# mnigm2001/Software-Defined-Radio

Measured on AMD Instinct MI355X. Metric: I/Q MS/s through front-end FIR+decimate+demod(+audio) per job; % HBM roofline, higher is better.
Workload: dtype i8+f32

## Files before the change

### software-defined-radio_amd/csrc/capi.hip

```cpp
#include "fmrx_internal.hpp"
#include "rds_station.hpp"
#include "build_id.hpp"

namespace fmrx {

static thread_local char g_err[512] = "";

void set_error(const char *fmt, ...)
{
    va_list ap;
    va_start(ap, fmt);
    vsnprintf(g_err, sizeof(g_err), fmt, ap);
    va_end(ap);
}

int fail(int code, const char *fmt, ...)
{
    va_list ap;
    va_start(ap, fmt);
    vsnprintf(g_err, sizeof(g_err), fmt, ap);
    va_end(ap);
    return code;
}

// ... 365 lines not shown
}

int fmrx_all_pass(const float *in, size_t n, float *state, size_t nstate, float *out)
{
    if (!in || !state || !out) return fail(FMRX_EINVAL, "all_pass: null buffer");
    if (n < nstate) return fail(FMRX_EINVAL, "all_pass: block of %zu samples shorter than the delay %zu", n, nstate);
    FMRX_TRY(require_device());
    Scratch &s = scratch();
    FMRX_TRY(s.a.ensure(n));
    FMRX_TRY(s.b.ensure(nstate));
    FMRX_TRY(s.c.ensure(n));
    FMRX_TRY(h2d(s.a.p, in, n * sizeof(float)));
    FMRX_TRY(h2d(s.b.p, state, nstate * sizeof(float)));
    FMRX_TRY(k_all_pass(s.a.p, n, s.b.p, nstate, s.c.p, nullptr));
    FMRX_TRY(d2h(out, s.c.p, n * sizeof(float)));
    std::memcpy(state, in + n - nstate, nstate * sizeof(float));
    return FMRX_OK;
}

int fmrx_fm_pll(const float *in, size_t n, float *nco_out, float *state, float freq, float Fs, float ncoScale,
                float phaseAdjust, float normBandwidth)
{
    if (!in || !nco_out || !state) return fail(FMRX_EINVAL, "fm_pll: null buffer");
    if (!(Fs > 0)) return fail(FMRX_EINVAL, "fm_pll: Fs must be positive");
    FMRX_TRY(require_device());
    Scratch &s = scratch();
    FMRX_TRY(s.a.ensure(n));
    FMRX_TRY(s.b.ensure(n + 1));
    FMRX_TRY(s.c.ensure(6));
    FMRX_TRY(h2d(s.a.p, in, n * sizeof(float)));
    FMRX_TRY(h2d(s.c.p, state, 6 * sizeof(float)));
    FMRX_TRY(k_fm_pll(s.a.p, n, s.b.p, s.c.p, freq, Fs, ncoScale, phaseAdjust, normBandwidth, 0, nullptr));
    FMRX_TRY(d2h(nco_out, s.b.p, (n + 1) * sizeof(float)));
    return d2h(state, s.c.p, 6 * sizeof(float));
}

int fmrx_stereo_mix(const float *stereo_filt, const float *pll, size_t n, float *mixer)
{
    if ((!stereo_filt || !pll || !mixer) && n) return fail(FMRX_EINVAL, "stereo_mix: null buffer");
    FMRX_TRY(require_device());
    Scratch &s = scratch();
    FMRX_TRY(s.a.ensure(n));
    FMRX_TRY(s.b.ensure(n));
    FMRX_TRY(s.c.ensure(n));
    FMRX_TRY(h2d(s.a.p, stereo_filt, n * sizeof(float)));
    FMRX_TRY(h2d(s.b.p, pll, n * sizeof(float)));
    FMRX_TRY(k_mix(s.a.p, s.b.p, n, s.c.p, nullptr));
    return d2h(mixer, s.c.p, n * sizeof(float));
}

int fmrx_stereo_combine(const float *stereo_final, const float *mono, size_t n, float *left, float *right)
{
    if ((!stereo_final || !mono || !left || !right) && n) return fail(FMRX_EINVAL, "stereo_combine: null buffer");
    FMRX_TRY(require_device());
    Scratch &s = scratch();
    FMRX_TRY(s.a.ensure(n));
    FMRX_TRY(s.b.ensure(n));
    FMRX_TRY(s.c.ensure(n));
    FMRX_TRY(s.d.ensure(n));
    FMRX_TRY(h2d(s.a.p, stereo_final, n * sizeof(float)));
    FMRX_TRY(h2d(s.b.p, mono, n * sizeof(float)));
    FMRX_TRY(k_combine(s.a.p, s.b.p, n, s.c.p, s.d.p, nullptr));
    FMRX_TRY(d2h(left, s.c.p, n * sizeof(float)));
    return d2h(right, s.d.p, n * sizeof(float));
}

int fmrx_diag_libm(int fn, const float *a, const float *b, size_t n, float *out)
{
    if (fn < 0 || fn > 5) return fail(FMRX_EINVAL, "diag_libm: fn must be 0 (sinf), 1 (cosf), 2 (atan2f) or 3..5 (their branch-free forms)");
    if ((!a || !out || (fn % 3 == 2 && !b)) && n) return fail(FMRX_EINVAL, "diag_libm: null buffer");
    FMRX_TRY(require_device());
    Scratch &s = scratch();
    FMRX_TRY(s.a.ensure(n));
    FMRX_TRY(s.b.ensure(n));
    FMRX_TRY(s.c.ensure(n));
    FMRX_TRY(h2d(s.a.p, a, n * sizeof(float)));
    if (fn % 3 == 2) FMRX_TRY(h2d(s.b.p, b, n * sizeof(float)));
    FMRX_TRY(k_libm_eval(fn, s.a.p, s.b.p, n, s.c.p, nullptr));
    return d2h(out, s.c.p, n * sizeof(float));
}

int fmrx_diag_stream_read_dev(const void *d_buf, size_t bytes, int method, void *stream)
{
    if (!d_buf || method < 0 || method > 4096) return fail(FMRX_EINVAL, "diag_stream_read_dev: bad arguments");
    FMRX_TRY(require_device());
    static thread_local DevBuf<unsigned> sink;
    FMRX_TRY(sink.ensure(4));
    return k_stream_read(d_buf, bytes, method, sink.p, static_cast<hipStream_t>(stream));
}

int fmrx_estimate_psd(float *freq, float *psd, const float *samples, size_t n, float Fs, int nfft)
{
    if (!freq || !psd || !samples) return fail(FMRX_EINVAL, "estimate_psd: null buffer");
    if (nfft < 2 || nfft % 2 || nfft > 65536) return fail(FMRX_EINVAL, "estimate_psd: nfft must be even and in 2..65536");
    if (n < static_cast<size_t>(nfft)) return fail(FMRX_EINVAL, "estimate_psd: %zu samples < nfft %d", n, nfft);
    if (!(Fs > 0)) return fail(FMRX_EINVAL, "estimate_psd: Fs must be positive");
    FMRX_TRY(require_device());
    Scratch &s = scratch();
    const size_t nseg = n / nfft, half = nfft / 2;
    FMRX_TRY(s.a.ensure(n));
    FMRX_TRY(s.b.ensure(nseg * half));
    FMRX_TRY(s.c.ensure(half));
    FMRX_TRY(s.d.ensure(half));
    FMRX_TRY(h2d(s.a.p, samples, nseg * nfft * sizeof(float)));
    FMRX_TRY(k_estimate_psd(s.a.p, n, Fs, nfft, s.b.p, s.c.p, s.d.p, nullptr));
    FMRX_TRY(d2h(freq, s.c.p, half * sizeof(float)));
    return d2h(psd, s.d.p, half * sizeof(float));
}

struct fmrx_fe_plan {
    FePlan plan;
};

int fmrx_fe_plan_create(fmrx_fe_plan **out, const float *h, size_t taps, unsigned decim)
{
    if (!out || !h) return fail(FMRX_EINVAL, "fe_plan_create: null argument");
    if (taps < 2 || taps > 65535) return fail(FMRX_EINVAL, "fe_plan_create: taps %zu not in 2..65535", taps);
    if (decim == 0) return fail(FMRX_EINVAL, "fe_plan_create: decim must be >= 1");
    FMRX_TRY(require_device());
    fmrx_fe_plan *p = new fmrx_fe_plan;
    int rc = fe_plan_init(p->plan, h, static_cast<int>(taps), static_cast<int>(decim));
    if (rc != FMRX_OK) {
        delete p;
        return rc;
    }
    *out = p;
    return FMRX_OK;
}

int fmrx_fe_plan_destroy(fmrx_fe_plan *plan)
{
    delete plan;
    return FMRX_OK;
}

int fmrx_fe_plan_is_specialised(const fmrx_fe_plan *plan) { return plan && plan->plan.fast ? 1 : 0; }
size_t fmrx_fe_plan_history_bytes(const fmrx_fe_plan *plan) { return plan ? plan->plan.hist_bytes : 0; }

int fmrx_fe_run_dev(const fmrx_fe_plan *plan, const uint8_t *d_iq, size_t n_samples, const uint8_t *d_hist, float *d_if,
                    int force_generic, void *stream)
{
    if (!plan || !d_iq || !d_if) return fail(FMRX_EINVAL, "fe_run_dev: null argument");
    return fe_launch(plan->plan, d_iq, n_samples, d_hist, d_if, default_options(), static_cast<hipStream_t>(stream),
                     force_generic != 0);
}

int fmrx_fe_fir_decim_u8(const uint8_t *iq, size_t n_samples, const float *h, size_t taps, unsigned decim, uint8_t *hist,
                         float *if_i, float *if_q, int force_generic)
{
    if (!iq || !h) return fail(FMRX_EINVAL, "fe_fir_decim_u8: null buffer");
    if (taps < 2 || taps > 65535) return fail(FMRX_EINVAL, "fe_fir_decim_u8: taps %zu not in 2..65535", taps);
    if (decim == 0) return fail(FMRX_EINVAL, "fe_fir_decim_u8: decim must be >= 1");
    if (hist && n_samples < taps - 1)
        return fail(FMRX_EINVAL, "fe_fir_decim_u8: block of %zu samples shorter than taps-1 = %zu", n_samples, taps - 1);
    FMRX_TRY(require_device());
    FePlan plan;
    FMRX_TRY(fe_plan_init(plan, h, static_cast<int>(taps), static_cast<int>(decim)));
    Scratch &s = scratch();
    const size_t n_out = n_samples / decim;
    const size_t hb = plan.hist_bytes, live = 2 * (taps - 1);
    FMRX_TRY(s.u.ensure(2 * n_samples));
    FMRX_TRY(s.uh.ensure(hb));
    FMRX_TRY(s.a.ensure(2 * n_out));
    FMRX_TRY(s.b.ensure(n_out));
    FMRX_TRY(s.c.ensure(n_out));
    FMRX_TRY(h2d(s.u.p, iq, 2 * n_samples));
    if (hist) {
// ... 88 lines not shown
```

### software-defined-radio_amd/csrc/kernels_diag.hip

```cpp
#include "fmrx_internal.hpp"

namespace fmrx {
namespace {

typedef unsigned u4 __attribute__((ext_vector_type(4)));

__global__ __launch_bounds__(256) void read_regs_kernel(const u4 *__restrict__ x, long n16, unsigned *__restrict__ out)
{
    const int lane = threadIdx.x & 63;
    const long waves = static_cast<long>(gridDim.x) * 4, w = static_cast<long>(blockIdx.x) * 4 + (threadIdx.x >> 6);
    const long pieces = n16 / 64;
    const long per = (pieces + waves - 1) / waves;
    const long p0 = w * per, p1 = p0 + per < pieces ? p0 + per : pieces;
    u4 acc = {0, 0, 0, 0};
    for (long p = p0; p < p1; p += 4) {
        u4 v[4];
#pragma unroll
        for (int i = 0; i < 4; i++) {
            const long q = p + i < p1 ? p + i : p1 - 1;
            v[i] = __builtin_nontemporal_load(x + q * 64 + lane);
        }
#pragma unroll
        for (int i = 0; i < 4; i++) acc ^= v[i];
    }
    if ((acc.x ^ acc.y ^ acc.z ^ acc.w) == 0x12345678u) out[0] = 1;
}

__global__ __launch_bounds__(256) void read_dma_kernel(const unsigned char *__restrict__ x, long n_bytes, unsigned *__restrict__ out, int SWEEP)
{
    extern __shared__ __attribute__((aligned(16))) unsigned char lds[];
    const int lane = threadIdx.x & 63, wave = threadIdx.x >> 6;
    unsigned char *ring = lds + wave * 4 * 3072;
    const long waves = static_cast<long>(gridDim.x) * 4, w = static_cast<long>(blockIdx.x) * 4 + wave;
    const long steps = n_bytes / 3072, per = (steps + waves - 1) / waves;
    const long s0 = w * per, s1 = s0 + per < steps ? s0 + per : steps;
    auto issue = [&](long s, int slot) {
        if (SWEEP) {
            const long i = s - s0, c = i / SWEEP, r = i - c * SWEEP;
            const long t = (c * waves + w) * SWEEP + r;
            s = t < steps ? t : steps - 1;
        }
#pragma unroll
        for (int k = 0; k < 3; k++)
            __builtin_amdgcn_global_load_lds((const __attribute__((address_space(1))) void *)(x + s * 3072 + k * 1024 + lane * 16),
                                             (__attribute__((address_space(3))) void *)(ring + slot * 3072 + k * 1024), 16, 0, 0);
    };
    u4 acc = {0, 0, 0, 0};
    for (int i = 0; i < 3 && s0 + i < s1; i++) issue(s0 + i, i);
    int slot = 0, fill = 3;
    for (long s = s0; s < s1; s++) {
        const bool steady = s + 3 < s1;
        if (steady) issue(s + 3, fill);
        if (steady) asm volatile("s_waitcnt vmcnt(9)" ::: "memory");
        else asm volatile("s_waitcnt vmcnt(0)" ::: "memory");
        const u4 *src = reinterpret_cast<const u4 *>(ring + slot * 3072);
        acc ^= src[lane] ^ src[64 + lane] ^ src[128 + lane];
        asm volatile("s_waitcnt lgkmcnt(0)" ::: "memory");
        slot = (slot + 1) & 3;
        fill = (fill + 1) & 3;
    }
    if ((acc.x ^ acc.y ^ acc.z ^ acc.w) == 0x12345678u) out[0] = 1;
}

}

int k_stream_read(const void *d_buf, size_t bytes, int method, unsigned *d_sink, hipStream_t s)
{
    if (bytes < 3072 * 1024) return fail(FMRX_EINVAL, "stream_read: buffer too small to mean anything");
    if (reinterpret_cast<uintptr_t>(d_buf) % 16) return fail(FMRX_EINVAL, "stream_read: buffer must be 16-byte aligned");
    if (method == 0)
        hipLaunchKernelGGL(read_regs_kernel, dim3(1024), dim3(256), 0, s, static_cast<const u4 *>(d_buf), static_cast<long>(bytes / 16), d_sink);
    else if (method == 1)
        hipLaunchKernelGGL(read_dma_kernel, dim3(512), dim3(256), 4 * 4 * 3072, s, static_cast<const unsigned char *>(d_buf),
                           static_cast<long>(bytes - bytes % 3072), d_sink, 0);
    else
        hipLaunchKernelGGL(read_dma_kernel, dim3(512), dim3(256), 4 * 4 * 3072, s, static_cast<const unsigned char *>(d_buf),
                           static_cast<long>(bytes - bytes % 3072), d_sink, method - 1);
    hipError_t e = hipGetLastError();
    if (e != hipSuccess) return fail(FMRX_EHIP, "launch stream_read: %s", hipGetErrorString(e));
    return FMRX_OK;
}

}
```

### software-defined-radio_amd/csrc/kernels_fe_mfma.hip

```cpp
#include "device_math.hpp"
#include "fe_mfma_host.hpp"
#include "fmrx_internal.hpp"

#include <cmath>
#include <type_traits>
#include <utility>

namespace fmrx {
namespace {

using i4 = int __attribute__((ext_vector_type(4)));
using f2 = float __attribute__((ext_vector_type(2)));
using f4 = float __attribute__((ext_vector_type(4)));

constexpr int iclamp(int v, int lo, int hi) { return v < lo ? lo : (v > hi ? hi : v); }

template <int T, int D, int PF = 0>
struct MfCfg {
    static constexpr int COL_OUT = 8;
    static constexpr int COLS = 16;
    static constexpr int TILE_OUT = COL_OUT * (COLS - 1);
    static constexpr int COL_BYTES = 2 * D * COL_OUT;
    static constexpr int STRIDE_BYTES = COL_BYTES * (COLS - 1);
    static constexpr int FRONT = (2 * (T - 1) + 15) / 16 * 16;
    static constexpr int WIN = FRONT + 2 * D * (COL_OUT - 1) + 2;
    static constexpr int KSTEPS = (WIN + 63) / 64;
    static constexpr int NDIG = kFeMfmaDigits;
    static constexpr int LEAD = COL_BYTES + FRONT;
    static constexpr int TILE_WIN = COL_BYTES * (COLS - 1) + 64 * KSTEPS;
    static constexpr int NPF = TILE_WIN / 1024;
    static constexpr int REM_LANES = (TILE_WIN % 1024) / 16;
    static constexpr int NP = NPF + (REM_LANES ? 1 : 0);
    static constexpr int SLOT = NP * 1024;
    static constexpr int P = PF ? PF : iclamp(8192 / TILE_WIN, 2, 8);
    static constexpr int NSLOT = P + 1;
    static constexpr int RING = NSLOT * SLOT;
    static_assert(TILE_WIN % 16 == 0 && COL_BYTES % 16 == 0, "16-byte fragments");
    static constexpr int YOUNGER = NP * P;
    static_assert(YOUNGER + 2 * P <= 63, "vmcnt is 6 bits");
};

template <class Fn, int... K>
__device__ __forceinline__ void for_each_index(std::integer_sequence<int, K...>, Fn &&f)
{
    (f(std::integral_constant<int, K>{}), ...);
}

template <int N>
__device__ __forceinline__ void wait_vmcnt()
{
    asm volatile("s_waitcnt vmcnt(%0)" ::"n"(N) : "memory");
}

template <int NPF, int REM_LANES>
__device__ __forceinline__ void dma_window(const uint8_t *__restrict__ x, const uint8_t *__restrict__ hist_end, long n_bytes,
                                           long s0, uint8_t *dst, int lane)
{
    constexpr int NP = NPF + (REM_LANES ? 1 : 0);
    if (s0 >= 0 && s0 + NP * 1024L <= n_bytes) {
        const uint8_t *base = x + s0;
#pragma unroll
        for (int k = 0; k < NP; k++)
            if (k < NPF || lane < REM_LANES)
                __builtin_amdgcn_global_load_lds((const __attribute__((address_space(1))) void *)(base + (lane * 16 + k * 1024)),
                                                 (__attribute__((address_space(3))) void *)(dst + k * 1024), 16, 0, 0);
    } else {
#pragma unroll
        for (int k = 0; k < NP; k++)
            if (k < NPF || lane < REM_LANES) {
                long off = s0 + k * 1024 + lane * 16;
                if (off > n_bytes - 16) off = n_bytes - 16;
                const uint8_t *src = off < 0 ? hist_end + off : x + off;
                __builtin_amdgcn_global_load_lds((const __attribute__((address_space(1))) void *)src,
                                                 (__attribute__((address_space(3))) void *)(dst + k * 1024), 16, 0, 0);
            }
    }
}

template <class C>
__device__ __forceinline__ void mf_dma_tile(const uint8_t *__restrict__ x, const uint8_t *__restrict__ hist_end, long n_bytes,
                                            int tile, uint8_t *ring, int rs, int lane)
{
    dma_window<C::NPF, C::REM_LANES>(x, hist_end, n_bytes, static_cast<long>(tile) * C::STRIDE_BYTES - C::LEAD,
                                     ring + rs * C::SLOT, lane);
}

template <int T, int D, int MINB, int PF>
__global__ __launch_bounds__(256, MINB) void fe_mfma_kernel(
    const uint8_t *__restrict__ x, const uint8_t *__restrict__ hist_end, long n_bytes, const i4 *__restrict__ a_img,
    float scale_lo, const float2 *__restrict__ prev_in, float *__restrict__ demod, float *__restrict__ y_if,
    float2 *__restrict__ prev_out, long n_out, int n_tiles, uint8_t *__restrict__ hist_next, int hist_bytes,
    const float *__restrict__ dhist_src, float *__restrict__ dhist_dst, int dhist_n)
{
    using C = MfCfg<T, D, PF>;
    extern __shared__ __attribute__((aligned(16))) uint8_t lds_raw[];
    const int lane = threadIdx.x & 63;
    const int wave = __builtin_amdgcn_readfirstlane(static_cast<int>(threadIdx.x >> 6));
    uint8_t *ring = lds_raw + wave * C::RING;
    const int tstep = static_cast<int>(gridDim.x) * 4;
    int tile = __builtin_amdgcn_readfirstlane(static_cast<int>(blockIdx.x) * 4 + wave);

    if (hist_next && tile == 0)
        for (int i = lane; i < hist_bytes; i += 64) hist_next[i] = x[n_bytes - hist_bytes + i];
    if (dhist_dst && tile == 1)
        for (int i = lane; i < dhist_n; i += 64) dhist_dst[i] = dhist_src[i];
    if (tile >= n_tiles) return;

    i4 a[C::KSTEPS][C::NDIG];
#pragma unroll
    for (int j = 0; j < C::KSTEPS; j++)
#pragma unroll
        for (int d = 0; d < C::NDIG; d++) a[j][d] = a_img[(j * C::NDIG + d) * 64 + lane];
    float ovi = 0.0f, ovq = 0.0f;
    const bool override_prev = prev_in != nullptr;
    if (override_prev) {
        const float2 p = *prev_in;
        ovi = p.x;
        ovq = p.y;
    }
    asm volatile("s_waitcnt vmcnt(0)" ::: "memory");
#pragma unroll
    for (int j = 0; j < C::KSTEPS; j++)
#pragma unroll
        for (int d = 0; d < C::NDIG; d++) asm volatile("" : "+v"(a[j][d]));
    asm volatile("" : "+v"(ovi), "+v"(ovq));

#pragma unroll
    for (int k = 0; k < C::P; k++)
        if (tile + k * tstep < n_tiles) mf_dma_tile<C>(x, hist_end, n_bytes, tile + k * tstep, ring, k, lane);

    const int col = lane & 15, g = lane >> 4;
    const int lane_off = C::COL_BYTES * col + 16 * g;
    const float scale_hi = scale_lo * 65536.0f;
    const bool with_if = y_if != nullptr;
    const int src_lane = lane >= 16 ? lane - 16 : lane + 47;
    int slot = 0, fill = C::P;
    auto fast_tile = [&](auto uc, auto modec, int t) {
        constexpr int u = decltype(uc)::value;
        constexpr int MODE = decltype(modec)::value;
        constexpr int FILL = (u + C::P) % C::NSLOT;
        {
            const uint8_t *src = x + (static_cast<long>(t + C::P * tstep) * C::STRIDE_BYTES - C::LEAD);
            uint8_t *dst = ring + FILL * C::SLOT;
#pragma unroll
            for (int q = 0; q < C::NP; q++)
                if (q < C::NPF || lane < C::REM_LANES)
                    __builtin_amdgcn_global_load_lds((const __attribute__((address_space(1))) void *)(src + (lane * 16 + q * 1024)),
                                                     (__attribute__((address_space(3))) void *)(dst + q * 1024), 16, 0, 0);
        }
        wait_vmcnt<C::YOUNGER + (MODE == 3 ? 2 : 1) * C::P>();
        __builtin_amdgcn_fence(__ATOMIC_ACQUIRE, "wavefront");
        __builtin_amdgcn_wave_barrier();
        const uint8_t *bsrc = ring + u * C::SLOT + lane_off;
        i4 b[C::KSTEPS];
#pragma unroll
        for (int j = 0; j < C::KSTEPS; j++) b[j] = *reinterpret_cast<const i4 *>(bsrc + 64 * j);
        __builtin_amdgcn_s_waitcnt(0xC07F);
// ... 164 lines not shown
        for (int d = 0; d < C::NDIG; d++) a[j][d] = a_img[(j * C::NDIG + d) * 64 + lane];
    asm volatile("s_waitcnt vmcnt(0)" ::: "memory");
#pragma unroll
    for (int j = 0; j < C::KSTEPS; j++)
#pragma unroll
        for (int d = 0; d < C::NDIG; d++) asm volatile("" : "+v"(a[j][d]));
    auto dma = [&](int t, int rs) {
        const int c = t / bk.tiles_per_row, j = t - c * bk.tiles_per_row;
        const long s0 = c * bk.in_pitch + bk.in_off + static_cast<long>(j) * C::STRIDE_BYTES - C::LEAD;
        dma_window<C::NPF, C::REM_LANES>(x, x, n_bytes, s0, ring + rs * C::SLOT, lane);
    };
#pragma unroll
    for (int k = 0; k < C::P; k++)
        if (tile + k * tstep < n_tiles) dma(tile + k * tstep, k);
    const int col = lane & 15, g = lane >> 4;
    const int lane_off = C::COL_BYTES * col + 16 * g;
    const float scale_hi = scale_lo * 65536.0f;
    const int src_lane = lane >= 16 ? lane - 16 : lane + 47;
    int slot = 0, fill = C::P;
    for (int it = 0; tile < n_tiles; tile += tstep, it++) {
        const bool steady = tile + C::P * tstep < n_tiles;
        if (steady) dma(tile + C::P * tstep, fill);
        if (steady) {
            if (it < C::P) wait_vmcnt<C::YOUNGER>();
            else wait_vmcnt<C::YOUNGER + C::P>();
        } else {
            wait_vmcnt<0>();
        }
        __builtin_amdgcn_fence(__ATOMIC_ACQUIRE, "wavefront");
        __builtin_amdgcn_wave_barrier();
        const uint8_t *bsrc = ring + slot * C::SLOT + lane_off;
        i4 b[C::KSTEPS];
#pragma unroll
        for (int j = 0; j < C::KSTEPS; j++) b[j] = *reinterpret_cast<const i4 *>(bsrc + 64 * j);
        __builtin_amdgcn_s_waitcnt(0xC07F);
        __builtin_amdgcn_fence(__ATOMIC_RELEASE, "wavefront");
        __builtin_amdgcn_wave_barrier();
        i4 acc[C::NDIG];
#pragma unroll
        for (int d = 0; d < C::NDIG; d++) acc[d] = (i4){0, 0, 0, 0};
#pragma unroll
        for (int j = 0; j < C::KSTEPS; j++) {
            const i4 bs = b[j] ^ static_cast<int>(0x80808080u);
#pragma unroll
            for (int d = 0; d < C::NDIG; d++) acc[d] = __builtin_amdgcn_mfma_i32_16x16x64_i8(a[j][d], bs, acc[d], 0, 0, 0);
        }
        float v[4];
#pragma unroll
        for (int k = 0; k < 4; k++) {
            int lo = acc[0][k];
            if (C::NDIG >= 2) lo += acc[1][k] * 256;
            const float flo = static_cast<float>(lo) * scale_lo;
            v[k] = C::NDIG >= 3 ? __builtin_fmaf(static_cast<float>(acc[2][k]), scale_hi, flo) : flo;
        }
        const float pi = __shfl(v[2], src_lane, 64), pq = __shfl(v[3], src_lane, 64);
        const float d0 = demod_fast(v[0], v[1], pi, pq), d1 = demod_fast(v[2], v[3], v[0], v[1]);
        const int c = tile / bk.tiles_per_row, j = tile - c * bk.tiles_per_row;
        const long ol = static_cast<long>(j) * C::TILE_OUT + C::COL_OUT * (col - 1) + 2 * g;
        if (col > 0 && ol < bk.n_row) *reinterpret_cast<f2 *>(demod + c * bk.out_pitch + bk.out_off + ol) = (f2){d0, d1};
        slot = slot + 1 == C::NSLOT ? 0 : slot + 1;
        fill = fill + 1 == C::NSLOT ? 0 : fill + 1;
    }
}

template <int T, int D, int TA, int DA>
struct FuCfg {
    using F = MfCfg<T, D>;
    static constexpr int TILE_OUT = 128;
    static constexpr int TILE_BYTES = F::COL_BYTES * 16;
    static constexpr int NPF = TILE_BYTES / 1024;
    static constexpr int REM_LANES = (TILE_BYTES % 1024) / 16;
    static constexpr int NP = NPF + (REM_LANES ? 1 : 0);
    static constexpr int P = iclamp(6144 / TILE_BYTES, 2, 8);
    static constexpr int NSLOT = P + 2;
    static constexpr int RING = NSLOT * TILE_BYTES;
    static constexpr int PIECE0 = NPF ? 1024 : TILE_BYTES;
    static_assert(F::WIN - F::COL_BYTES <= PIECE0, "window overlap must fit the next slot's first piece");
    static_assert(64 * F::KSTEPS - F::COL_BYTES <= RING - TILE_BYTES, "K padding laps the ring");
    static constexpr int YOUNGER = (NP - 1) + NP * P;
    static_assert(YOUNGER <= 63, "vmcnt is 6 bits");
    static constexpr int AB_OUT = 256;
    static constexpr int TB = AB_OUT * DA / TILE_OUT;
    static_assert(TB * TILE_OUT == AB_OUT * DA, "batches end on tile boundaries");
    static constexpr int AWIN = (TA - 1) + 15 * DA + 1;
    static constexpr int AK = (AWIN + 15) / 16 * 4;
    static_assert(AK % 4 == 0 && (TA - 1) % 4 == 0, "window in whole 16-byte groups");
    static constexpr int KPT = ((AK + TB - 3) / (TB - 2) + 3) / 4 * 4;
    static constexpr int NPH = (AK + KPT - 1) / KPT;
    static constexpr int DR_MIN = AB_OUT * DA + TA - 1 + (4 * AK - AWIN) + (NPH + 1) * TILE_OUT;
    static constexpr int DR = (DR_MIN + TILE_OUT - 1) / TILE_OUT * TILE_OUT;
    static_assert(NPH <= TB - 2, "a batch must be done before the next one completes");
    static_assert(AB_OUT * DA + TA - 1 + (4 * AK - AWIN) + (NPH + 1) * TILE_OUT <= DR, "ring too small for the delayed multiply");
    static_assert(DR % TILE_OUT == 0, "tiles must not wrap inside");
    static_assert(TA - 1 <= TILE_OUT - 1, "one dry tile must cover the audio history");
    static constexpr int MIRROR = 4 * KPT;
    static_assert(MIRROR <= TILE_OUT, "the mirror is refreshed by the tile at position 0");
    static constexpr int LDS_WAVE = RING + (DR + MIRROR) * 4;
};

template <class C, class F>
__device__ __forceinline__ void fu_dma_slot(const uint8_t *__restrict__ x, const uint8_t *__restrict__ hist_end, long n_bytes,
                                            int u, uint8_t *ring, int rs, int lane)
{
    dma_window<C::NPF, C::REM_LANES>(x, hist_end, n_bytes, static_cast<long>(u) * C::TILE_BYTES - F::FRONT,
                                     ring + rs * C::TILE_BYTES, lane);
}

template <int T, int D, int TA, int DA>
__global__ __launch_bounds__(256, 2) void mono_fused_kernel(
    const uint8_t *__restrict__ x, const uint8_t *__restrict__ hist_end, long n_bytes, const i4 *__restrict__ a_img,
    float scale_lo, const float *__restrict__ au_img, const float2 *__restrict__ prev_in,
    const float *__restrict__ dhist_end, float *__restrict__ demod_tail, int tail_keep, float2 *__restrict__ prev_out,
    float *__restrict__ audio, int16_t *__restrict__ pcm, int wrap, long n_out, int n_tiles, long n_audio, int n_batches,
    int batches_per_wave, uint8_t *__restrict__ hist_next, int hist_bytes)
{
    using C = FuCfg<T, D, TA, DA>;
    using F = typename C::F;
    extern __shared__ __attribute__((aligned(16))) uint8_t lds_raw[];
    const int lane = threadIdx.x & 63;
    const int wave = __builtin_amdgcn_readfirstlane(static_cast<int>(threadIdx.x >> 6));
    uint8_t *ring = lds_raw + wave * C::LDS_WAVE;
    float *dring = reinterpret_cast<float *>(ring + C::RING);
    const int wid = __builtin_amdgcn_readfirstlane(static_cast<int>(blockIdx.x) * 4 + wave);

    if (hist_next && wid == 0)
        for (int i = lane; i < hist_bytes; i += 64) hist_next[i] = x[n_bytes - hist_bytes + i];

    const int b0 = wid * batches_per_wave;
    const int b1 = b0 + batches_per_wave < n_batches ? b0 + batches_per_wave : n_batches;
    if (b0 >= b1) return;
    const int t0 = b0 * C::TB;
    const int t1 = b1 * C::TB < n_tiles ? b1 * C::TB : n_tiles;
    const int tb = t0 > 0 ? t0 - 1 : 0;

    i4 a[F::KSTEPS][F::NDIG];
#pragma unroll
    for (int j = 0; j < F::KSTEPS; j++)
#pragma unroll
        for (int d = 0; d < F::NDIG; d++) a[j][d] = a_img[(j * F::NDIG + d) * 64 + lane];
    float au[C::AK];
#pragma unroll
    for (int j = 0; j < C::AK; j++) au[j] = au_img[j * 64 + lane];
    float ci = 0.0f, cq = 0.0f;
    for (int i = lane; i < C::DR + C::MIRROR; i += 64) dring[i] = 0.0f;
    if (t0 == 0) {
        const float2 p = *prev_in;
        ci = p.x;
        cq = p.y;
        for (int i = lane; i < TA - 1; i += 64) dring[C::TILE_OUT - (TA - 1) + i] = dhist_end[i - (TA - 1)];
    }
    asm volatile("s_waitcnt vmcnt(0) lgkmcnt(0)" ::: "memory");
#pragma unroll
    for (int j = 0; j < F::KSTEPS; j++)
#pragma unroll
        for (int d = 0; d < F::NDIG; d++) asm volatile("" : "+v"(a[j][d]));
#pragma unroll
    for (int j = 0; j < C::AK; j++) asm volatile("" : "+v"(au[j]));
    asm volatile("" : "+v"(ci), "+v"(cq));

    {
        int rs = 0;
        for (int u = tb; u <= tb + C::P && u <= t1; u++) {
            fu_dma_slot<C, F>(x, hist_end, n_bytes, u, ring, rs, lane);
            rs++;
        }
    }

    const int col = lane & 15, g = lane >> 4;
    const int lane_off = F::COL_BYTES * col + 16 * g;
    const float scale_hi = scale_lo * 65536.0f;
    const int src_lane = lane >= 16 ? lane - 16 : lane + 47;
    int wrap_adr[F::KSTEPS];
#pragma unroll
    for (int j = 0; j < F::KSTEPS; j++) {
        const int adr = (C::NSLOT - 1) * C::TILE_BYTES + lane_off + 64 * j;
        wrap_adr[j] = adr >= C::RING ? adr - C::RING : adr;
    }
    int slot = 0, fill = C::P + 1;
    int dpos = C::TILE_OUT;
    bool pend = false;
    int pend_ph = 0, pend_ws = 0;
    long pend_a0 = 0;
    f4 y0 = (f4){0.0f, 0.0f, 0.0f, 0.0f}, y1 = y0;
    f4 xs[C::KPT / 4];
    auto slice_load = [&]() {
#pragma unroll
        for (int k = 0; k < C::KPT / 4; k++)
            xs[k] = *reinterpret_cast<const f4 *>(dring + pend_ws + 16 * k);
        pend_ws += 4 * C::KPT;
        pend_ws = pend_ws >= C::DR ? pend_ws - C::DR : pend_ws;
    };
    auto slice_mfma = [&]() {
#pragma unroll
        for (int ph = 0; ph < C::NPH; ph++)
            if (pend_ph == ph) {
#pragma unroll
                for (int j = ph * C::KPT; j < (ph + 1) * C::KPT && j < C::AK; j++) {
                    const float xv = xs[(j - ph * C::KPT) / 4][j % 4];
                    if (j & 1) y1 = __builtin_amdgcn_mfma_f32_16x16x4f32(au[j], xv, y1, 0, 0, 0);
                    else y0 = __builtin_amdgcn_mfma_f32_16x16x4f32(au[j], xv, y0, 0, 0, 0);
                }
            }
    };
    auto store_batch = [&]() {
        const f4 y = y0 + y1;
        const long ao = pend_a0 + 4 * g;
        if (ao + 3 < n_audio) {
            if (audio) *reinterpret_cast<f4 *>(audio + ao) = y;
            if (pcm) {
                using s4 = short __attribute__((ext_vector_type(4)));
                const s4 pk = (s4){pcm_pack_flat(y[0], wrap), pcm_pack_flat(y[1], wrap), pcm_pack_flat(y[2], wrap), pcm_pack_flat(y[3], wrap)};
                *reinterpret_cast<s4 *>(pcm + ao) = pk;
            }
        } else {
#pragma unroll
            for (int k = 0; k < 4; k++)
                if (ao + k < n_audio) {
                    if (audio) audio[ao + k] = y[k];
                    if (pcm) pcm[ao + k] = pcm_pack(y[k], wrap);
                }
        }
    };
    auto slice_done = [&]() {
        pend_ph++;
        if (pend_ph == C::NPH) {
            store_batch();
            pend = false;
        }
    };
    auto begin_batch = [&](int bt) {
        pend = true;
        pend_ph = 0;
        pend_a0 = static_cast<long>(bt) * C::AB_OUT + 16 * col;
        int sb = (bt * C::AB_OUT * DA - (TA - 1)) - (C::TILE_OUT * tb - C::TILE_OUT);
        pend_ws = (sb + 16 * col * DA + 4 * g) % C::DR;
        y0 = (f4){0.0f, 0.0f, 0.0f, 0.0f};
        y1 = y0;
    };
    int t_fast1 = 0;
    bool fast_last = false;
    if (scale_lo >= 8.8817842e-16f) {
        const long in_x = (n_bytes - C::NP * 1024L + F::FRONT) / C::TILE_BYTES;
        const long no_tail = (n_out - tail_keep) / C::TILE_OUT - 1;
        long lim = t1 - C::P - 1;
        lim = lim < in_x - C::P - 1 ? lim : in_x - C::P - 1;
        lim = lim < no_tail ? lim : no_tail;
        t_fast1 = lim + 1 >= C::TB ? static_cast<int>((lim + 1) / C::TB) * C::TB : 0;
        fast_last = t1 % C::TB == 0 && t1 - C::TB >= t0 && t1 <= in_x && t1 - 1 <= no_tail;
    }
    auto fast_tile = [&](auto kc, auto lastc, int t) {
        constexpr int k = decltype(kc)::value;
        constexpr bool STEADY = !decltype(lastc)::value || k + C::P + 1 <= C::TB;
        constexpr int WAIT = STEADY ? C::YOUNGER : (C::NP - 1) + C::NP * (C::TB - k - 1);
        auto slice_k = [&]() {
#pragma unroll
            for (int j = k * C::KPT; j < (k + 1) * C::KPT && j < C::AK; j++) {
                const float xv = xs[(j - k * C::KPT) / 4][j % 4];
                if (j & 1) y1 = __builtin_amdgcn_mfma_f32_16x16x4f32(au[j], xv, y1, 0, 0, 0);
                else y0 = __builtin_amdgcn_mfma_f32_16x16x4f32(au[j], xv, y0, 0, 0, 0);
            }
        };
        if constexpr (STEADY) {
            const uint8_t *src = x + (static_cast<long>(t + C::P + 1) * C::TILE_BYTES - F::FRONT);
            uint8_t *dst = ring + fill * C::TILE_BYTES;
#pragma unroll
            for (int q = 0; q < C::NP; q++)
                if (q < C::NPF || lane < C::REM_LANES)
                    __builtin_amdgcn_global_load_lds((const __attribute__((address_space(1))) void *)(src + (lane * 16 + q * 1024)),
                                                     (__attribute__((address_space(3))) void *)(dst + q * 1024), 16, 0, 0);
        }
        wait_vmcnt<WAIT>();
        __builtin_amdgcn_fence(__ATOMIC_ACQUIRE, "wavefront");
        __builtin_amdgcn_wave_barrier();
        i4 b[F::KSTEPS];
        if (slot != C::NSLOT - 1) {
            const uint8_t *bsrc = ring + slot * C::TILE_BYTES + lane_off;
#pragma unroll
            for (int j = 0; j < F::KSTEPS; j++) b[j] = *reinterpret_cast<const i4 *>(bsrc + 64 * j);
        } else {
#pragma unroll
            for (int j = 0; j < F::KSTEPS; j++) b[j] = *reinterpret_cast<const i4 *>(ring + wrap_adr[j]);
        }
        if constexpr (k < C::NPH) slice_load();
        __builtin_amdgcn_s_waitcnt(0xC07F);
        __builtin_amdgcn_fence(__ATOMIC_RELEASE, "wavefront");
        __builtin_amdgcn_wave_barrier();
        i4 acc[F::NDIG];
#pragma unroll
        for (int d = 0; d < F::NDIG; d++) acc[d] = (i4){0, 0, 0, 0};
#pragma unroll
        for (int j = 0; j < F::KSTEPS; j++) {
            const i4 bs = b[j] ^ static_cast<int>(0x80808080u);
#pragma unroll
            for (int d = 0; d < F::NDIG; d++) acc[d] = __builtin_amdgcn_mfma_i32_16x16x64_i8(a[j][d], bs, acc[d], 0, 0, 0);
        }
        float v[4];
#pragma unroll
        for (int q = 0; q < 4; q++) {
            int lo = acc[0][q];
            if (F::NDIG >= 2) lo += acc[1][q] * 256;
            const float flo = static_cast<float>(lo) * scale_lo;
            v[q] = F::NDIG >= 3 ? __builtin_fmaf(static_cast<float>(acc[2][q]), scale_hi, flo) : flo;
        }
        float pi = __shfl(v[2], src_lane, 64), pq = __shfl(v[3], src_lane, 64);
        pi = lane == 0 ? ci : pi;
        pq = lane == 0 ? cq : pq;
        ci = __builtin_bit_cast(float, __builtin_amdgcn_readlane(__builtin_bit_cast(int, v[2]), 63));
        cq = __builtin_bit_cast(float, __builtin_amdgcn_readlane(__builtin_bit_cast(int, v[3]), 63));
        const float d0 = demod_fast_bounded(v[0], v[1], pi, pq);
        const float d1 = demod_fast_bounded(v[2], v[3], v[0], v[1]);
        const int ol = F::COL_OUT * col + 2 * g;
        *reinterpret_cast<f2 *>(dring + dpos + ol) = (f2){d0, d1};
        if (dpos == 0 && ol < C::MIRROR) *reinterpret_cast<f2 *>(dring + C::DR + ol) = (f2){d0, d1};
        slot = slot + 1 == C::NSLOT ? 0 : slot + 1;
        fill = fill + 1 == C::NSLOT ? 0 : fill + 1;
        dpos = dpos + C::TILE_OUT == C::DR ? 0 : dpos + C::TILE_OUT;
        if constexpr (k < C::NPH) slice_k();
        if constexpr (k == C::NPH - 1) store_batch();
    };
    for (int t = tb;;) {
        if (t >= t0 && (t < t_fast1 || (fast_last && t == t1 - C::TB)) && t % C::TB == 0 && (!pend || pend_ph == 0)) {
            if (!pend) {
                begin_batch(t / C::TB);
                pend_a0 = n_audio;
            }
            for (; t < t_fast1; t += C::TB) {
                for_each_index(std::make_integer_sequence<int, C::TB>{},
                               [&](auto kc) { fast_tile(kc, std::false_type{}, t + decltype(kc)::value); });
                begin_batch(t / C::TB);
            }
            if (fast_last && t == t1 - C::TB) {
                for_each_index(std::make_integer_sequence<int, C::TB>{},
                               [&](auto kc) { fast_tile(kc, std::true_type{}, t + decltype(kc)::value); });
                begin_batch(t / C::TB);
                t += C::TB;
            }
        }
        const bool have_tile = t < t1;
        bool completed = false;
        if (have_tile) {
            const bool sl = pend;
            const bool steady = t + C::P + 1 <= t1;
            if (steady) fu_dma_slot<C, F>(x, hist_end, n_bytes, t + C::P + 1, ring, fill, lane);
            if (steady) wait_vmcnt<C::YOUNGER>();
            else wait_vmcnt<0>();
            __builtin_amdgcn_fence(__ATOMIC_ACQUIRE, "wavefront");
            __builtin_amdgcn_wave_barrier();

            i4 b[F::KSTEPS];
            if (slot != C::NSLOT - 1) {
                const uint8_t *bsrc = ring + slot * C::TILE_BYTES + lane_off;
#pragma unroll
                for (int j = 0; j < F::KSTEPS; j++) b[j] = *reinterpret_cast<const i4 *>(bsrc + 64 * j);
            } else {
#pragma unroll
                for (int j = 0; j < F::KSTEPS; j++) b[j] = *reinterpret_cast<const i4 *>(ring + wrap_adr[j]);
            }
            if (sl) slice_load();
            __builtin_amdgcn_s_waitcnt(0xC07F);
            __builtin_amdgcn_fence(__ATOMIC_RELEASE, "wavefront");
            __builtin_amdgcn_wave_barrier();

            i4 acc[F::NDIG];
#pragma unroll
            for (int d = 0; d < F::NDIG; d++) acc[d] = (i4){0, 0, 0, 0};
#pragma unroll
            for (int j = 0; j < F::KSTEPS; j++) {
                const i4 bs = b[j] ^ static_cast<int>(0x80808080u);
#pragma unroll
                for (int d = 0; d < F::NDIG; d++)
                    acc[d] = __builtin_amdgcn_mfma_i32_16x16x64_i8(a[j][d], bs, acc[d], 0, 0, 0);
            }
            float v[4];
#pragma unroll
            for (int k = 0; k < 4; k++) {
                int lo = acc[0][k];
                if (F::NDIG >= 2) lo += acc[1][k] * 256;
                const float flo = static_cast<float>(lo) * scale_lo;
                v[k] = F::NDIG >= 3 ? __builtin_fmaf(static_cast<float>(acc[2][k]), scale_hi, flo) : flo;
            }
            float pi = __shfl(v[2], src_lane, 64), pq = __shfl(v[3], src_lane, 64);
            if (lane == 0) {
                pi = ci;
                pq = cq;
            }
            ci = __builtin_bit_cast(float, __builtin_amdgcn_readlane(__builtin_bit_cast(int, v[2]), 63));
            cq = __builtin_bit_cast(float, __builtin_amdgcn_readlane(__builtin_bit_cast(int, v[3]), 63));
            const float d0 = demod_fast(v[0], v[1], pi, pq);
            const float d1 = demod_fast(v[2], v[3], v[0], v[1]);

            const int ol = F::COL_OUT * col + 2 * g;
            const long o = static_cast<long>(t) * C::TILE_OUT + ol;
            *reinterpret_cast<f2 *>(dring + dpos + ol) = (f2){d0, d1};
            if (dpos == 0 && ol < C::MIRROR) *reinterpret_cast<f2 *>(dring + C::DR + ol) = (f2){d0, d1};
            if (t >= t0 && static_cast<long>(t + 1) * C::TILE_OUT > n_out - tail_keep &&
                o + 2 > n_out - tail_keep && o < n_out) {
                if (demod_tail && o >= n_out - tail_keep) demod_tail[o] = d0;
                if (demod_tail && o + 1 < n_out) demod_tail[o + 1] = d1;
                if (prev_out && o + 2 == n_out) *prev_out = make_float2(v[2], v[3]);
                if (prev_out && o + 1 == n_out) *prev_out = make_float2(v[0], v[1]);
            }
            slot = slot + 1 == C::NSLOT ? 0 : slot + 1;
            fill = fill + 1 == C::NSLOT ? 0 : fill + 1;
            dpos = dpos + C::TILE_OUT == C::DR ? 0 : dpos + C::TILE_OUT;
            if (sl) {
                slice_mfma();
                slice_done();
            }
            completed = t >= t0 && ((t + 1) % C::TB == 0 || t + 1 == n_tiles);
            t++;
        }

        while (pend && (completed || !have_tile)) {
            slice_load();
            slice_mfma();
            slice_done();
        }
        if (completed) begin_batch((t - 1) / C::TB);
        if (!have_tile && !pend) break;
// ... 173 lines not shown
```

Baseline: 2.590 million.

## Use non-temporal buffer LDS-DMA loads with compile-time ring slots in fast path

Switches the front-end's global-to-LDS DMA loads to a non-temporal cache policy (aux=2) and uses buffer-resource loads with scalar offsets in the fast tile path. Ring slot indices are tied to the absolute tile number, so each batch can be specialized on its starting slot and all LDS read and fill offsets become compile-time constants, removing the runtime wrap branch. A sched_barrier is added, and the diagnostic stream-read kernel gains a non-temporal variant. The cost is larger code from multiple batch instantiations, and the non-temporal hint may hurt if the halo overlap between tiles relied on cache reuse.

```diff
diff --git a/software-defined-radio_amd/csrc/capi.hip b/software-defined-radio_amd/csrc/capi.hip
--- a/software-defined-radio_amd/csrc/capi.hip
+++ b/software-defined-radio_amd/csrc/capi.hip
@@ -471,7 +471,7 @@
 
 int fmrx_diag_stream_read_dev(const void *d_buf, size_t bytes, int method, void *stream)
 {
-    if (!d_buf || method < 0 || method > 4096) return fail(FMRX_EINVAL, "diag_stream_read_dev: bad arguments");
+    if (!d_buf || method < 0 || (method & ~0x10000) > 4096) return fail(FMRX_EINVAL, "diag_stream_read_dev: bad arguments");
     FMRX_TRY(require_device());
     static thread_local DevBuf<unsigned> sink;
     FMRX_TRY(sink.ensure(4));
diff --git a/software-defined-radio_amd/csrc/kernels_diag.hip b/software-defined-radio_amd/csrc/kernels_diag.hip
--- a/software-defined-radio_amd/csrc/kernels_diag.hip
+++ b/software-defined-radio_amd/csrc/kernels_diag.hip
@@ -26,6 +26,7 @@
     if ((acc.x ^ acc.y ^ acc.z ^ acc.w) == 0x12345678u) out[0] = 1;
 }
 
+template <int AUX>
 __global__ __launch_bounds__(256) void read_dma_kernel(const unsigned char *__restrict__ x, long n_bytes, unsigned *__restrict__ out, int SWEEP)
 {
     extern __shared__ __attribute__((aligned(16))) unsigned char lds[];
@@ -43,7 +44,7 @@
 #pragma unroll
         for (int k = 0; k < 3; k++)
             __builtin_amdgcn_global_load_lds((const __attribute__((address_space(1))) void *)(x + s * 3072 + k * 1024 + lane * 16),
-                                             (__attribute__((address_space(3))) void *)(ring + slot * 3072 + k * 1024), 16, 0, 0);
+                                             (__attribute__((address_space(3))) void *)(ring + slot * 3072 + k * 1024), 16, 0, AUX);
     };
     u4 acc = {0, 0, 0, 0};
     for (int i = 0; i < 3 && s0 + i < s1; i++) issue(s0 + i, i);
@@ -68,14 +69,18 @@
 {
     if (bytes < 3072 * 1024) return fail(FMRX_EINVAL, "stream_read: buffer too small to mean anything");
     if (reinterpret_cast<uintptr_t>(d_buf) % 16) return fail(FMRX_EINVAL, "stream_read: buffer must be 16-byte aligned");
-    if (method == 0)
+    const bool nt = (method & 0x10000) != 0;
+    const int m = method & 0xffff;
+    if (nt && m == 0) return fail(FMRX_EINVAL, "stream_read: the non-temporal variant is of the LDS-DMA methods");
+    const int sweep = m >= 2 ? m - 1 : 0;
+    if (m == 0)
         hipLaunchKernelGGL(read_regs_kernel, dim3(1024), dim3(256), 0, s, static_cast<const u4 *>(d_buf), static_cast<long>(bytes / 16), d_sink);
-    else if (method == 1)
-        hipLaunchKernelGGL(read_dma_kernel, dim3(512), dim3(256), 4 * 4 * 3072, s, static_cast<const unsigned char *>(d_buf),
-                           static_cast<long>(bytes - bytes % 3072), d_sink, 0);
+    else if (nt)
+        hipLaunchKernelGGL(read_dma_kernel<2>, dim3(512), dim3(256), 4 * 4 * 3072, s, static_cast<const unsigned char *>(d_buf),
+                           static_cast<long>(bytes - bytes % 3072), d_sink, sweep);
     else
-        hipLaunchKernelGGL(read_dma_kernel, dim3(512), dim3(256), 4 * 4 * 3072, s, static_cast<const unsigned char *>(d_buf),
-                           static_cast<long>(bytes - bytes % 3072), d_sink, method - 1);
+        hipLaunchKernelGGL(read_dma_kernel<0>, dim3(512), dim3(256), 4 * 4 * 3072, s, static_cast<const unsigned char *>(d_buf),
+                           static_cast<long>(bytes - bytes % 3072), d_sink, sweep);
     hipError_t e = hipGetLastError();
     if (e != hipSuccess) return fail(FMRX_EHIP, "launch stream_read: %s", hipGetErrorString(e));
     return FMRX_OK;
diff --git a/software-defined-radio_amd/csrc/kernels_fe_mfma.hip b/software-defined-radio_amd/csrc/kernels_fe_mfma.hip
--- a/software-defined-radio_amd/csrc/kernels_fe_mfma.hip
+++ b/software-defined-radio_amd/csrc/kernels_fe_mfma.hip
@@ -13,7 +13,10 @@
 using f2 = float __attribute__((ext_vector_type(2)));
 using f4 = float __attribute__((ext_vector_type(4)));
 
+constexpr int kNtPolicy = 2;
+
 constexpr int iclamp(int v, int lo, int hi) { return v < lo ? lo : (v > hi ? hi : v); }
+constexpr int igcd(int a, int b) { return b == 0 ? a : igcd(b, a % b); }
 
 template <int T, int D, int PF = 0>
 struct MfCfg {
@@ -52,7 +55,7 @@
     asm volatile("s_waitcnt vmcnt(%0)" ::"n"(N) : "memory");
 }
 
-template <int NPF, int REM_LANES>
+template <int NPF, int REM_LANES, int AUX = 0>
 __device__ __forceinline__ void dma_window(const uint8_t *__restrict__ x, const uint8_t *__restrict__ hist_end, long n_bytes,
                                            long s0, uint8_t *dst, int lane)
 {
@@ -63,7 +66,7 @@
         for (int k = 0; k < NP; k++)
             if (k < NPF || lane < REM_LANES)
                 __builtin_amdgcn_global_load_lds((const __attribute__((address_space(1))) void *)(base + (lane * 16 + k * 1024)),
-                                                 (__attribute__((address_space(3))) void *)(dst + k * 1024), 16, 0, 0);
+                                                 (__attribute__((address_space(3))) void *)(dst + k * 1024), 16, 0, AUX);
     } else {
 #pragma unroll
         for (int k = 0; k < NP; k++)
@@ -72,7 +75,7 @@
                 if (off > n_bytes - 16) off = n_bytes - 16;
                 const uint8_t *src = off < 0 ? hist_end + off : x + off;
                 __builtin_amdgcn_global_load_lds((const __attribute__((address_space(1))) void *)src,
-                                                 (__attribute__((address_space(3))) void *)(dst + k * 1024), 16, 0, 0);
+                                                 (__attribute__((address_space(3))) void *)(dst + k * 1024), 16, 0, AUX);
             }
     }
 }
@@ -403,6 +406,9 @@
     static constexpr int AB_OUT = 256;
     static constexpr int TB = AB_OUT * DA / TILE_OUT;
     static_assert(TB * TILE_OUT == AB_OUT * DA, "batches end on tile boundaries");
+    static constexpr int SLOT_STEP = igcd(TB, NSLOT);
+    static constexpr int NSTART = NSLOT / SLOT_STEP;
+    static constexpr int LANE_OFF_END = F::COL_BYTES * (F::COLS - 1) + 16 * 3 + 16;
     static constexpr int AWIN = (TA - 1) + 15 * DA + 1;
     static constexpr int AK = (AWIN + 15) / 16 * 4;
     static_assert(AK % 4 == 0 && (TA - 1) % 4 == 0, "window in whole 16-byte groups");
@@ -423,8 +429,8 @@
 __device__ __forceinline__ void fu_dma_slot(const uint8_t *__restrict__ x, const uint8_t *__restrict__ hist_end, long n_bytes,
                                             int u, uint8_t *ring, int rs, int lane)
 {
-    dma_window<C::NPF, C::REM_LANES>(x, hist_end, n_bytes, static_cast<long>(u) * C::TILE_BYTES - F::FRONT,
-                                     ring + rs * C::TILE_BYTES, lane);
+    dma_window<C::NPF, C::REM_LANES, kNtPolicy>(x, hist_end, n_bytes, static_cast<long>(u) * C::TILE_BYTES - F::FRONT,
+                                                ring + rs * C::TILE_BYTES, lane);
 }
 
 template <int T, int D, int TA, int DA>
@@ -479,13 +485,7 @@
     for (int j = 0; j < C::AK; j++) asm volatile("" : "+v"(au[j]));
     asm volatile("" : "+v"(ci), "+v"(cq));
 
-    {
-        int rs = 0;
-        for (int u = tb; u <= tb + C::P && u <= t1; u++) {
-            fu_dma_slot<C, F>(x, hist_end, n_bytes, u, ring, rs, lane);
-            rs++;
-        }
-    }
+    for (int u = tb; u <= tb + C::P && u <= t1; u++) fu_dma_slot<C, F>(x, hist_end, n_bytes, u, ring, u % C::NSLOT, lane);
 
     const int col = lane & 15, g = lane >> 4;
     const int lane_off = F::COL_BYTES * col + 16 * g;
@@ -497,7 +497,7 @@
         const int adr = (C::NSLOT - 1) * C::TILE_BYTES + lane_off + 64 * j;
         wrap_adr[j] = adr >= C::RING ? adr - C::RING : adr;
     }
-    int slot = 0, fill = C::P + 1;
+    int slot = tb % C::NSLOT, fill = (tb + C::P + 1) % C::NSLOT;
     int dpos = C::TILE_OUT;
     bool pend = false;
     int pend_ph = 0, pend_ws = 0;
@@ -569,8 +569,17 @@
         t_fast1 = lim + 1 >= C::TB ? static_cast<int>((lim + 1) / C::TB) * C::TB : 0;
         fast_last = t1 % C::TB == 0 && t1 - C::TB >= t0 && t1 <= in_x && t1 - 1 <= no_tail;
     }
-    auto fast_tile = [&](auto kc, auto lastc, int t) {
+    int t_cur = tb;
+    const long rbase = static_cast<long>(tb) * C::TILE_BYTES;
+    const long reach = static_cast<long>(t1 - tb + 1) * C::TILE_BYTES + C::NP * 1024L;
+    const __amdgpu_buffer_rsrc_t xr = __builtin_amdgcn_make_buffer_rsrc(
+        const_cast<uint8_t *>(x + rbase), 0, static_cast<int>(reach < n_bytes - rbase ? reach : n_bytes - rbase), 0x00020000);
+    const int lane16 = 16 * lane;
+    const uint8_t *lring = ring + lane_off;
+    auto fast_tile = [&](auto kc, auto lastc, auto sc, int t) {
         constexpr int k = decltype(kc)::value;
+        constexpr int U = (decltype(sc)::value + k) % C::NSLOT;
+        constexpr int FILL = (U + C::P + 1) % C::NSLOT;
         constexpr bool STEADY = !decltype(lastc)::value || k + C::P + 1 <= C::TB;
         constexpr int WAIT = STEADY ? C::YOUNGER : (C::NP - 1) + C::NP * (C::TB - k - 1);
         auto slice_k = [&]() {
@@ -582,27 +591,31 @@
             }
         };
         if constexpr (STEADY) {
-            const uint8_t *src = x + (static_cast<long>(t + C::P + 1) * C::TILE_BYTES - F::FRONT);
-            uint8_t *dst = ring + fill * C::TILE_BYTES;
-#pragma unroll
-            for (int q = 0; q < C::NP; q++)
+            const int soff = (t + C::P + 1 - tb) * C::TILE_BYTES - F::FRONT;
+            for_each_index(std::make_integer_sequence<int, C::NP>{}, [&](auto qc) {
+                constexpr int q = decltype(qc)::value;
                 if (q < C::NPF || lane < C::REM_LANES)
-                    __builtin_amdgcn_global_load_lds((const __attribute__((address_space(1))) void *)(src + (lane * 16 + q * 1024)),
-                                                     (__attribute__((address_space(3))) void *)(dst + q * 1024), 16, 0, 0);
+                    __builtin_amdgcn_raw_ptr_buffer_load_lds(
+                        xr, (__attribute__((address_space(3))) void *)(ring + FILL * C::TILE_BYTES + q * 1024), 16, lane16,
+                        soff + q * 1024, 0, kNtPolicy);
+            });
         }
         wait_vmcnt<WAIT>();
         __builtin_amdgcn_fence(__ATOMIC_ACQUIRE, "wavefront");
         __builtin_amdgcn_wave_barrier();
         i4 b[F::KSTEPS];
-        if (slot != C::NSLOT - 1) {
-            const uint8_t *bsrc = ring + slot * C::TILE_BYTES + lane_off;
-#pragma unroll
-            for (int j = 0; j < F::KSTEPS; j++) b[j] = *reinterpret_cast<const i4 *>(bsrc + 64 * j);
-        } else {
-#pragma unroll
-            for (int j = 0; j < F::KSTEPS; j++) b[j] = *reinterpret_cast<const i4 *>(ring + wrap_adr[j]);
-        }
+        for_each_index(std::make_integer_sequence<int, F::KSTEPS>{}, [&](auto jc) {
+            constexpr int j = decltype(jc)::value;
+            constexpr int OFF = U * C::TILE_BYTES + 64 * j;
+            if constexpr (OFF + C::LANE_OFF_END > C::RING) {
+                static_assert(U == C::NSLOT - 1, "only the last slot wraps");
+                b[j] = *reinterpret_cast<const i4 *>(ring + wrap_adr[j]);
+            } else {
+                b[j] = *reinterpret_cast<const i4 *>(lring + OFF);
+            }
+        });
         if constexpr (k < C::NPH) slice_load();
+        __builtin_amdgcn_sched_barrier(0);
         __builtin_amdgcn_s_waitcnt(0xC07F);
         __builtin_amdgcn_fence(__ATOMIC_RELEASE, "wavefront");
         __builtin_amdgcn_wave_barrier();
@@ -633,29 +646,32 @@
         const int ol = F::COL_OUT * col + 2 * g;
         *reinterpret_cast<f2 *>(dring + dpos + ol) = (f2){d0, d1};
         if (dpos == 0 && ol < C::MIRROR) *reinterpret_cast<f2 *>(dring + C::DR + ol) = (f2){d0, d1};
-        slot = slot + 1 == C::NSLOT ? 0 : slot + 1;
-        fill = fill + 1 == C::NSLOT ? 0 : fill + 1;
         dpos = dpos + C::TILE_OUT == C::DR ? 0 : dpos + C::TILE_OUT;
         if constexpr (k < C::NPH) slice_k();
         if constexpr (k == C::NPH - 1) store_batch();
     };
-    for (int t = tb;;) {
+    auto fast_batch = [&](auto lastc) {
+        const int s0 = t_cur % C::NSLOT;
+        for_each_index(std::make_integer_sequence<int, C::NSTART>{}, [&](auto ic) {
+            constexpr int S = decltype(ic)::value * C::SLOT_STEP;
+            if (s0 == S)
+                for_each_index(std::make_integer_sequence<int, C::TB>{}, [&](auto kc) {
+                    fast_tile(kc, lastc, std::integral_constant<int, S>{}, t_cur + decltype(kc)::value);
+                });
+        });
+        begin_batch(t_cur / C::TB);
+        t_cur += C::TB;
+    };
+    for (int &t = t_cur;;) {
         if (t >= t0 && (t < t_fast1 || (fast_last && t == t1 - C::TB)) && t % C::TB == 0 && (!pend || pend_ph == 0)) {
             if (!pend) {
                 begin_batch(t / C::TB);
                 pend_a0 = n_audio;
             }
-            for (; t < t_fast1; t += C::TB) {
-                for_each_index(std::make_integer_sequence<int, C::TB>{},
-                               [&](auto kc) { fast_tile(kc, std::false_type{}, t + decltype(kc)::value); });
-                begin_batch(t / C::TB);
-            }
-            if (fast_last && t == t1 - C::TB) {
-                for_each_index(std::make_integer_sequence<int, C::TB>{},
-                               [&](auto kc) { fast_tile(kc, std::true_type{}, t + decltype(kc)::value); });
-                begin_batch(t / C::TB);
-                t += C::TB;
-            }
+            while (t < t_fast1) fast_batch(std::false_type{});
+            if (fast_last && t == t1 - C::TB) fast_batch(std::true_type{});
+            slot = t % C::NSLOT;
+            fill = (t + C::P + 1) % C::NSLOT;
         }
         const bool have_tile = t < t1;
         bool completed = false;
```

Measured after the change: 2.758 million, median of 6. 6.5% higher.
